# ishovkun/poroelasticity-dealii

Hardware: AMD Instinct MI355X
Metric: DoF-updates/sec in assemble+SpMV per fixed-stress iter (higher is better)
Workload: dtype f64

## Files before the change

poroelasticity_dealii_amd/csrc/common.hpp:

```cpp
#pragma once
#include <hip/hip_runtime.h>
#include <cstdint>
#include <cstdio>
#include <map>
#include <memory>
#include <type_traits>
#include <stdexcept>
#include <string>
#include <list>
#include <vector>
#include "../../include/poroel_hip.h"
#include "fdm_tables.hpp"
#include "cell_field.hpp"

namespace poro {

#define PORO_HIP(x)                                                                                   \
  do { hipError_t e_ = (x); if (e_ != hipSuccess) throw poro::Error(std::string(#x) + " -> " + hipGetErrorString(e_)); } while (0)

template <class T> struct DevBuf {
  T *p = nullptr; size_t n = 0;
  DevBuf() = default; DevBuf(const DevBuf &) = delete; DevBuf &operator=(const DevBuf &) = delete;
  ~DevBuf() { release(); }
  void release() { if (p) (void)hipFree(p); p = nullptr; n = 0; }
// ... 43 lines not shown
};
struct FdmDist : SlabLayout {
  bool built = false;
  FdmDir last;
  DevBuf<double> sendbuf, recvbuf, tz1, tz2; std::vector<double> hsend, hrecv;
  DevBuf<FdmWindow> windows;
};

struct FdmuDir { int n = 0; bool reg_form = false, split = false, blk = false; int n_even = 0; int blk_kk[2] = {0, 0}, blk_nch[2] = {0, 0}, blk_mb[2] = {0, 0} ; DevBuf<double> fwd, bwd, lam; };
struct FdmU : SlabLayout {
              int dim = 0; int nn[3] = {1, 1, 1}; double coef[3][3] = {}; FdmuDir dir[3][3]; FdmuDir last_global[3]; bool built = false, single = false;
              int fix[3][3][2] = {};
              bool dist = false; DevBuf<double> sendbuf, recvbuf, tz1, tz2;
              bool line = false; DevBuf<double> line_coef, line_fac; };
struct FdmoPlans;
struct FdmOct {
  bool built = false; int nt = 0;
  int n[3] = {1, 1, 1}, h[3] = {1, 1, 1}; int hxp = 2;
  int64_t co_stride = 0, n_oct = 0;
  double coef[3][3] = {};
  DevBuf<double> fwd[3][3][2], bwd[3][3][2], lam[3][3][2];
  DevBuf<float> fwd32[3][3][2], bwd32[3][3][2];
  DevBuf<double> g, z, t;
  DevBuf<double> gz_part; int gz_n = 0;
  std::vector<double> h_lam[3][3][2];
  DevBuf<double> bxy;
  int no = 8;
  int nc = 3;
  bool planar = false;
  int own_z = 0;
// ... 2 lines not shown
    bool on = false; int n_ranks = 1, rank = 0;
    int ng = 0, hzg = 0;
    bool zboth = false; DevBuf<int64_t> dst2;
    int np = 2, nb = 12;
    int cw = 64, nchunk = 0, cps = 0, chunk0 = 0, my_chunks = 0;
    int64_t scols = 0;
    int own = 0, nl = 0, max_own = 0, max_nl = 0, rows_back = 0;
    int64_t recv_off = 0;
    DevBuf<int64_t> row_in;
    DevBuf<int64_t> row_out; DevBuf<int32_t> row_kz;
    DevBuf<double> buf, tz;
  } slab;
  std::shared_ptr<FdmoPlans> plans;
  struct ScalarTable { double a, kappa; DevBuf<double> t; };
  std::list<ScalarTable> scalar_tables;
};
struct FdmQ1 { FdmScalar nodal; FdmOct fused; };
struct SsorLevels { DevBuf<int32_t> fwd_rows, bwd_rows; std::vector<int64_t> fwd_off, bwd_off; bool built = false; };
struct CsrDev {
  int64_t n = 0, nnz = 0;
  DevBuf<int64_t> rp; DevBuf<int32_t> col; DevBuf<int64_t> diag_pos;
  int lanes_per_row = 8;
  SsorLevels ssor;
};

struct ConsDev {
  int64_t n = 0, n_masters = 0;
  DevBuf<int32_t> dof, master; DevBuf<int64_t> ptr; DevBuf<double> weight, inhom;
  DevBuf<int32_t> t_master, t_dof; DevBuf<int64_t> t_ptr; DevBuf<double> t_weight;
  DevBuf<uint8_t> inert;
// ... 125 lines not shown

namespace poro {

inline bool box_fast_u(const poro_ctx *c) { return c->box.enabled && !c->mod.kind; }
inline bool moduli_structured_applies(const poro_ctx *c) {
  return c->box.enabled && c->dim == 3 && (c->k_u == 1 || c->k_u == 2) && c->mod.kind == 1 && c->operator_mode == PORO_OP_MATRIX_FREE && c->mf_variant == 1 && !c->comm.multi() &&
         c->comm.part.n_ranks <= 1;
}
inline bool moduli_structured(const poro_ctx *c) { return c->moduli_op == PORO_MODULI_OP_STRUCTURED && c->mod.planes.p && moduli_structured_applies(c); }

void la_fill(hipStream_t s, double *x, double v, int64_t n);
void la_nodal_interp(hipStream_t s, const int64_t *ptr, const int32_t *col, const double *w, int64_t n_rows, int ncomp, const double *in, double *out, int lanes = 1);
void la_two_level_combine(hipStream_t s, const int64_t *ptr, const int32_t *col, const double *w, int64_t n_rows, int ncomp, const double *zc, const double *g, const double *dinv, const uint8_t *inert, double omega, double *z, int lanes = 1);
void la_copy_many(hipStream_t s, int count, double *const *dst, const double *const *src, const int64_t *n);
void la_post(hipStream_t s, Mailbox *mb, unsigned long long seq, const double *src, int n, const PcgScalars *sc);
void la_copy(hipStream_t s, double *y, const double *x, int64_t n);
void la_axpy(hipStream_t s, double *y, double a, const double *x, int64_t n);
void la_add_range(hipStream_t s, double *y, const double *x, int64_t n);
void la_add_two_ranges(hipStream_t s, double *y0, const double *x0, double *y1, const double *x1, int64_t n);
void la_dot_partials(hipStream_t s, const double *a, const double *b, int64_t n, double *partials , const PcgScalars *gate = nullptr );
void la_norm_partials(hipStream_t s, const double *a, int64_t n, double *partials_l2, double *partials_inf);
void la_reduce_finish(hipStream_t s, const double *partials, int n_sets, double *red , int max_not_sum_mask);
void la_csr_spmv(hipStream_t s, const CsrDev &A, const double *val, const double *x, double *y);
void la_csr_residual(hipStream_t s, const CsrDev &A, const double *M, const double *K, double kappa, const double *t, const double *p,
                     const double *src, double *R);
void la_pressure_tmp(hipStream_t s, double *t, const double *ev, const double *ev0, const double *p, const double *p_old, double c1, double c2, int64_t n);
void la_jacobian(hipStream_t s, double *J, const double *M, const double *K, double a, double kappa, int64_t nnz);
void la_ifc_pack(hipStream_t s, const IfcDev &I, const double *v);
void la_ifc_sum(hipStream_t s, const IfcDev &I, double *v);
void la_csr_diag(hipStream_t s, const CsrDev &A, const double *val, double *diag);
// ... 97 lines not shown
void fdmu_line_factor(hipStream_t s, int ku, int ncomp, const FdmuLineArgs &a, double *fac );
void fdmu_line_solve(hipStream_t s, int ku, int ncomp, const FdmuLineArgs &a, const double *fac, double *v );
bool fdmo_usable(int dim, const int nn[3]);
void fdmo_init(FdmOct &O, const int nn[3], const double coef[3][3], hipStream_t s);
void fdmo_init_slab(FdmOct &O, const int nn[3], const double coef[3][3], int rank, const std::vector<int> &node_layers, bool has_upper, hipStream_t s);
void fdmo_init_per_direction(FdmOct &O, const int nn[3], const double coef[3][3], const FdmFormDecision &D, hipStream_t s);
void fdmo_upload_dir(FdmOct &O, int comp, int dir, const LineTables &T);
void fdmo_finalize(FdmOct &O);
void fdmo_apply(hipStream_t s, const FdmOct &O, const double *g_oct, double *z_oct, double *scratch_oct, const PcgScalars *gate = nullptr, hipEvent_t *ev  = nullptr,
                double *gz_part  = nullptr,
                int precision  = PORO_FDM_FP64,
                const PcgStopTest &stop = PcgStopTest{} );
bool fdmo_scalar_usable(int dim, const int nn[3]);
void fdmo_scalar_init(FdmOct &O, const int nn[3], hipStream_t s);
void fdmo_scalar_upload_dir(FdmOct &O, int dir, const LineTables &T);
void fdmo_scalar_apply(hipStream_t s, FdmOct &O, double a, double kappa, const double *g, double *z, const PcgScalars *gate = nullptr);
void fdmo_scalar_apply_many(hipStream_t s, FdmOct &O, double a, double kappa, int nb, const double *const *g, double *const *z, const PcgScalars *gate = nullptr);
void la_residual_norms_many(hipStream_t s, int nb, const double *const *y, const double *const *b, int64_t n, double *partials, const uint8_t *mask = nullptr);
void fdmo_scalar_init_slab(FdmOct &O, const int nn[3], int rank, const std::vector<int> &node_layers, hipStream_t s);
void fdmo_scalar_slab_pass(hipStream_t s, FdmOct &O, int pass, double a, double kappa, const double *in, double *out);
bool fdmo_planar_usable(int dim, const int nn[3]);
void fdmo_init_planar(FdmOct &O, const int nn[3], const double coef[3][3], hipStream_t s, bool split = true );
void fdmo_upload_dir_planar(FdmOct &O, int comp, int dir, const LineTables &T);
void fdmo_apply_planar(hipStream_t s, const FdmOct &O, const double *g_q, double *z_q, const PcgScalars *gate = nullptr, const PcgStopTest &stop = PcgStopTest{} );
void fdmo_from_nodal(hipStream_t s, const FdmOct &O, const double *v_nodal, double *q_oct);
void fdmo_to_nodal(hipStream_t s, const FdmOct &O, const double *r_oct, double *v_nodal);
void fdmo_init_residual(hipStream_t s, const FdmOct &O, double *g_oct, const double *Ax, const double *b, const uint8_t *inert);
void fdmo_first_direction(hipStream_t s, const FdmOct &O, double *d, const double *g_oct, const double *z_oct, double *partials );
void fdmo_update_g(hipStream_t s, const FdmOct &O, PcgScalars *sc, int parity, double *g_oct, const double *h, const uint8_t *inert, const double *partials_dh, double *partials_out , const double *red = nullptr);
void fdmo_update_d(hipStream_t s, const FdmOct &O, PcgScalars *sc, int parity, int it, double *x, double *d, const double *z_oct, const double *partials_in , const double *red = nullptr,
                   bool gz_from_pass = false ,
                   bool stream_x = false ,
// ... 19 lines not shown
```

poroelasticity_dealii_amd/csrc/ctx.hip:

```cpp
#include <dlfcn.h>
#include <rccl/rccl.h>
#include <algorithm>
#include <array>
#include <chrono>
#include <cmath>
#include <cstdlib>
#include <cstring>
#include <functional>
#include <thread>
#include <unordered_map>
#include "common.hpp"
#include "ctx_internal.hpp"

using namespace poro;
using namespace poro::ctx_detail;

namespace {
void lifting_from_wh(poro_ctx *c) {
  la_fill(c->stream, c->lift_u.p, 0.0, c->n_u);
  la_axpy(c->stream, c->lift_u.p, -1.0, c->wh_u.p, c->n_u);
}

void throw_unless_close(poro_ctx *c, double *a, const double *b, int64_t n, double rel_tol, const char *what) {
  hipStream_t s = c->stream;
// ... 313 lines not shown
  bool distribute_inhom = true;
};

const uint8_t *proj_inert(poro_ctx *c) { return c->cons_p.hanging.p ? c->cons_p.hanging.p : c->cons_p.inert.p; }

bool q1_stencil(poro_ctx *c) { return c->operator_mode == PORO_OP_MATRIX_FREE && c->box.enabled; }

bool solve_q1_direct(poro_ctx *c, double a, double kappa, int n, const double *const *b, double *const *x, double *y_scratch, bool batched,
                     const poro_solver_opts *opts, poro_solve_info *info, Q1Set set = Q1Set::free_ends, const uint8_t *mask = nullptr, const double *kap = nullptr, int kap_ncomp = 0) {
  hipStream_t s = c->stream;
  const double *y[3];
  for (int e = 0; e < n; ++e) y[e] = y_scratch + (size_t)e * c->n_p;
  const auto t0 = std::chrono::steady_clock::now();
  if (batched) {
    Timed tm(c, "precondition_p_fdm");
    fdmo_scalar_apply_many(s, c->q1_free.fused, a, kappa, n, b, x);
  } else {
    const double kk[3] = {kappa, kappa, kappa};
    for (int e = 0; e < n; ++e) { if (kap) fdm_precondition_p_layered(c, a, b[e], x[e], set); else fdm_precondition_p(c, a, kk, b[e], x[e], set); }
  }
  for (int e = 0; e < n; ++e) {
    {
      Timed tm(c, "apply_p_stencil");
      if (kap) p_stencil_apply_var(s, c->dim, c->box, a, kap, kap_ncomp, x[e], const_cast<double *>(y[e]));
      else p_stencil_apply(s, c->dim, c->box, a, kappa, x[e], const_cast<double *>(y[e]));
    }
    exchange_add(c, const_cast<double *>(y[e]), c->n_p, c->comm.part.plane_p);
  }
  la_residual_norms_many(s, n, y, b, owned(c, c->n_p, c->comm.part.plane_p), c->partials.p, mask);
  pcg_scalars_sum(s, c->partials.p, 2 * n, c->red.p);
  allreduce_sum(c, c->red.p, 2 * n);
  post_and_wait(c, c->red.p, 2 * n);
  bool all = true;
  for (int e = 0; e < n; ++e) {
    const double res = std::sqrt(c->mailbox->vals[2 * e]), bn = std::sqrt(c->mailbox->vals[2 * e + 1]);
    const bool ok = res <= std::max(opts->abs_tol, opts->rel_tol * bn);
    all = all && ok;
    if (!info) continue;
    info[e] = poro_solve_info{};
    info[e].iterations = 0;
    info[e].converged = ok ? 1 : 0;
    info[e].initial_residual = bn;
    info[e].final_residual = res;
    info[e].operator_applications = 1;
    info[e].seconds = std::chrono::duration<double>(std::chrono::steady_clock::now() - t0).count() / n;
  }
  return all;
// ... 332 lines not shown
    PORO_HIP(hipMemcpyAsync(host, vec(c, which), n * sizeof(double), hipMemcpyDeviceToHost, c->stream)); PORO_HIP(hipStreamSynchronize(c->stream)); return 0;
  });
}
int poro_vec_fill(poro_ctx *c, int which, double v) { return guarded([&] { PORO_HIP(hipSetDevice(c->device)); la_fill(c->stream, vec(c, which), v, vec_len(c, which)); return 0; }); }
int poro_vec_copy(poro_ctx *c, int dst, int src) {
  return guarded([&] { PORO_HIP(hipSetDevice(c->device)); if (vec_len(c, dst) != vec_len(c, src)) throw Error("vector length mismatch"); la_copy(c->stream, vec(c, dst), vec(c, src), vec_len(c, dst)); return 0; });
}
int poro_vec_axpy(poro_ctx *c, int y, double a, int x) {
  return guarded([&] { PORO_HIP(hipSetDevice(c->device)); if (vec_len(c, y) != vec_len(c, x)) throw Error("vector length mismatch"); la_axpy(c->stream, vec(c, y), a, vec(c, x), vec_len(c, y)); return 0; });
}
int poro_vec_norm(poro_ctx *c, int which, double *l2, double *linf) {
  return guarded([&] {
    PORO_HIP(hipSetDevice(c->device));
    const int64_t n = vec_len(c, which), plane = is_u_vec(which) ? c->comm.part.plane_u : c->comm.part.plane_p;
    la_norm_partials(c->stream, vec(c, which), owned(c, n, plane), c->partials.p, c->partials.p + kMaxPartials);
    la_reduce_finish(c->stream, c->partials.p, 2, c->red.p, 2);
    allreduce_sum(c, c->red.p, 1);
    post_and_wait(c, c->red.p, 2);
    if (l2) *l2 = std::sqrt(c->mailbox->vals[0]); if (linf) *linf = c->mailbox->vals[1]; return 0;
  });
}

int poro_state_save(poro_ctx *c) {
  return guarded([&] {
    PORO_HIP(hipSetDevice(c->device));
    std::vector<double *> dst; std::vector<const double *> src; std::vector<int64_t> len;
    for (auto &kv : c->vec) { DevBuf<double> &d = c->vec_saved[kv.first]; if (d.n != kv.second.n) d.alloc(kv.second.n); dst.push_back(d.p); src.push_back(kv.second.p); len.push_back((int64_t)kv.second.n); }
    la_copy_many(c->stream, (int)dst.size(), dst.data(), src.data(), len.data());
    PORO_HIP(hipStreamSynchronize(c->stream)); return 0;
  });
}
int poro_state_restore(poro_ctx *c) {
  return guarded([&] {
// ... 105 lines not shown
    PORO_HIP(hipSetDevice(c->device));
    hipStream_t s = c->stream; double *R = vec(c, PORO_VEC_RESIDUAL_P);
    const double *src = c->grav.flux_on() ? c->grav.src_p.p : c->src_local.p;
    {
      Timed tm(c, "pressure_residual");
      la_pressure_tmp(s, c->tmp_p.p, vec(c, PORO_VEC_EPSV), vec(c, PORO_VEC_EPSV0), vec(c, PORO_VEC_P), vec(c, PORO_VEC_P_OLD), c->mat.biot_alpha / dt, 1. / c->mat.biot_M / dt, c->n_p);
      if (c->operator_mode == PORO_OP_MATRIX_FREE && c->box.enabled) {
        if (c->perm.kind) p_residual_stencil_var(s, c->dim, c->box, c->perm.lattice.p, c->perm.ncomp, c->tmp_p.p, vec(c, PORO_VEC_P), src, R);
        else p_residual_stencil(s, c->dim, c->box, c->mat.k_over_mu, c->tmp_p.p, vec(c, PORO_VEC_P), src, R);
      } else la_csr_residual(s, c->Ap, c->Mp.p, c->Kp.p, c->perm.kind ? 1.0 : c->mat.k_over_mu, c->tmp_p.p, vec(c, PORO_VEC_P), src, R);
    }
    la_cons_reduce(s, c->cons_p, R);
    exchange_add(c, R, c->n_p, c->comm.part.plane_p);
    if (c->n_pdir) la_mask_zero(s, R, c->pdir_mask.p, c->n_p);
    la_dot_partials(s, R, R, owned(c, c->n_p, c->comm.part.plane_p), c->partials.p);
    la_reduce_finish(s, c->partials.p, 1, c->red.p, 0);
    allreduce_sum(c, c->red.p, 1);
    post_and_wait(c, c->red.p, 1);
    if (l2) *l2 = std::sqrt(c->mailbox->vals[0]);
    return 0;
  });
}

int poro_pres_apply_boundary_values(poro_ctx *c) {
  return guarded([&] {
    PORO_HIP(hipSetDevice(c->device));
    if (c->n_pdir) la_set_constrained(c->stream, vec(c, PORO_VEC_P), c->pdir_mask.p, c->pdir_val.p, c->n_p);
    if (c->n_pdir && c->cons_p.n) {
      la_cons_expand(c->stream, c->cons_p, vec(c, PORO_VEC_P), true);
      la_set_constrained(c->stream, vec(c, PORO_VEC_P), c->pdir_mask.p, c->pdir_val.p, c->n_p);
    }
    return 0;
  });
// ... 267 lines not shown
```

poroelasticity_dealii_amd/csrc/ctx_comm.hip:

```cpp
#include <dlfcn.h>
#include <rccl/rccl.h>
#include <algorithm>
#include <array>
#include <chrono>
#include <cmath>
#include <cstdlib>
#include <cstring>
#include <functional>
#include <thread>
#include <unordered_map>
#include "common.hpp"
#include "ctx_internal.hpp"

using namespace poro;
using namespace poro::ctx_detail;

namespace poro {
namespace ctx_detail {
thread_local std::string g_err;

Rccl g_rccl;
void Rccl::load() {
  if (lib) return;
  lib = dlopen("librccl.so.1", RTLD_NOW | RTLD_GLOBAL);
// ... 27 lines not shown
  }
}
static void isolate_sampled_dispatch(poro_ctx *c) {
  if (c->timing_stride <= 1) return;
  hipEvent_t m = event_get(c); (void)hipEventRecord(m, c->stream); c->event_pool.push_back(m);
}
Timer *begin_sampled_dispatch(poro_ctx *c, const char *family) {
  if (!c->timing) return nullptr;
  Timer *t = &c->timers[family];
  if (!t->sample(c->timing_stride)) return nullptr;
  isolate_sampled_dispatch(c);
  return t;
}


void post_and_wait(poro_ctx *c, const double *dev_src, int n, const PcgScalars *sc) {
  if (n > 16) throw Error("post_and_wait: at most 16 scalars");
  const unsigned long long want = ++c->mb_seq;
  la_post(c->stream, c->mailbox, want, dev_src, n, sc);
  PORO_HIP(hipGetLastError());
  const auto t0 = std::chrono::steady_clock::now(); unsigned spins = 0;
  while (__atomic_load_n(const_cast<unsigned long long *>(&c->mailbox->seq), __ATOMIC_ACQUIRE) != want) {
    __builtin_ia32_pause();
    if ((++spins & 0xfffff) == 0) {
      const hipError_t q = hipStreamQuery(c->stream);
      if (q != hipSuccess && q != hipErrorNotReady) throw Error(std::string("device failed while the host waited for its answer: ") + hipGetErrorString(q));
      if (q == hipSuccess && __atomic_load_n(const_cast<unsigned long long *>(&c->mailbox->seq), __ATOMIC_ACQUIRE) != want) throw Error("mailbox: the stream drained without publishing the expected sequence number");
      if (std::chrono::duration<double>(std::chrono::steady_clock::now() - t0).count() > 600.0) throw Error("mailbox: no answer from the device within 600 s");
    }
  }
}

void build_interface(poro_ctx *c, IfcDev &I, const int64_t *ptr, const int32_t *dof, int64_t n, int64_t n_owned) {
  const poro_partition &pt = c->comm.part; const int nn = pt.n_neighbours;
// ... 222 lines not shown
```

poroelasticity_dealii_amd/csrc/ctx_internal.hpp:

```cpp
#pragma once
#include <rccl/rccl.h>
#include <functional>
#include <string>
#include <vector>
#include "common.hpp"
#include "whole_faces.hpp"
#include "fdm_tables.hpp"

namespace poro {
namespace ctx_detail {

extern thread_local std::string g_err;
inline int ipow(int b, int e) { int r = 1; while (e--) r *= b; return r; }
template <class F> int guarded(F &&f) {
  try { return f(); }
  catch (const std::exception &e) { g_err = e.what(); return -1; }
}
template <class F> void for_each_colour(poro_ctx *c, F &&fn) {
  for (size_t k = 0; k + 1 < c->color_off.size(); ++k)
    fn(c->color_cells.p + c->color_off[k], c->color_off[k + 1] - c->color_off[k]);
}

struct Rccl {
  void *lib = nullptr;
// ... 23 lines not shown
  Timer *t = begin_sampled_dispatch(c, family);
  if (!t) return launch(nullptr, nullptr);
  hipEvent_t e0 = event_get(c), e1 = event_get(c);
  auto r = launch(e0, e1);
  t->pending.emplace_back(e0, e1);
  t->launches++;
  return r;
}
struct EventPair {
  poro_ctx *c; hipEvent_t e0, e1;
  explicit EventPair(poro_ctx *c_) : c(c_), e0(event_get(c_)), e1(event_get(c_)) {}
  ~EventPair() { c->event_pool.push_back(e0); c->event_pool.push_back(e1); }
  EventPair(const EventPair &) = delete; EventPair &operator=(const EventPair &) = delete;
};
void post_and_wait(poro_ctx *c, const double *dev_src, int n, const PcgScalars *sc = nullptr);

void setup_general_partition(poro_ctx *c, const poro_desc *d);
void exchange_planes(poro_ctx *c, const double *send_lo, const double *send_hi, int64_t plane);
void exchange_add(poro_ctx *c, double *v, int64_t n, int64_t plane);
void allreduce_sum(poro_ctx *c, double *dev, int n);
void allreduce_sum_vec(poro_ctx *c, double *dev, int64_t n, const char *timer);
int64_t owned(poro_ctx *c, int64_t n, int64_t plane);
AsmArgs asm_args(poro_ctx *c);
MfArgs mf_args(poro_ctx *c);
void mf_operator(poro_ctx *c, const double *x, double *y, bool constrained);
void mfg_operator(poro_ctx *c, const double *x, double *y, bool constrained);
void build_spatial_cells(poro_ctx *c);
void assemble_loads_u(poro_ctx *c);
void sync_moduli_planes(poro_ctx *c);
void hybrid_enable(poro_ctx *c);
// ... 76 lines not shown
```

poroelasticity_dealii_amd/csrc/ctx_prec.hip:

```cpp
#include <dlfcn.h>
#include <rccl/rccl.h>
#include <algorithm>
#include <array>
#include <chrono>
#include <cmath>
#include <cstdlib>
#include <cstring>
#include <functional>
#include <new>
#include <optional>
#include <thread>
#include <unordered_map>
#include "common.hpp"
#include "ctx_internal.hpp"
#include "perm_line.hpp"
#include "moduli_line.hpp"

using namespace poro;
using namespace poro::ctx_detail;

namespace poro {
namespace ctx_detail {
bool fdm_p_supported(poro_ctx *c) {
  if (!c->lines.on) return false;
// ... 58 lines not shown
  F.windows.upload(W);
  F.built = true;
}
void build_fdm_q1(poro_ctx *c, Q1Set which) {
  const bool fixed = which == Q1Set::fixed_ends;
  FdmQ1 &T = q1_set(c, which);
  if (T.nodal.built) return;
  if (fixed) {
    if (!fdm_pj_supported(c)) throw Error("PORO_PREC_FDM with prescribed pressures needs a uniform box or tensor-product grid on one rank whose prescribed set is a union of whole faces");
    if (c->timing) c->timers["fdm_pj_build"].enqueued += 1;
  } else if (!fdm_p_supported(c)) throw Error("PORO_PREC_FDM needs a uniform box (poro_desc.box.enabled) and, when partitioned, an initialised communicator");
  T.nodal.dim = c->dim;
  const bool multi = !fixed && c->comm.multi();
  int np3[3] = {c->lines.n[0] + 1, c->lines.n[1] + 1, c->dim == 3 ? c->lines.n[2] + 1 : 1};
  const bool fused = !multi && fdmo_scalar_usable(c->dim, np3) && !std::getenv("PORO_FDM_P_UNFUSED");
  if (fused) fdmo_scalar_init(T.fused, np3, c->stream);
  for (int d = 0; d < c->dim; ++d) {
    const std::vector<double> &hcell = c->lines.hcell[d]; const bool lo = fixed && c->pdir_face[d][0], hi = fixed && c->pdir_face[d][1];
    upload_dir(T.nodal.dir[d], c->lines.uniform && !lo && !hi ? q1_eig((int)hcell.size(), hcell[0]) : line_tables(1, hcell, lo, hi), fused ? &T.fused : nullptr, d);
  }
  if (!multi) T.fused.built = fused;
  if (c->fdm_t1.n < (size_t)c->n_p) { c->fdm_t1.alloc(c->n_p); c->fdm_t2.alloc(c->n_p); }
  if (multi) build_fdm_dist(c, np3);
  T.nodal.built = true;
}
void alltoall_blocks(poro_ctx *c, double *send, double *recv, int64_t blk, bool self_in_place) {
  Comm &cm = c->comm; const int N = cm.part.n_ranks, r = cm.part.rank;
  Timed tm(c, "alltoall");
  if (!self_in_place) PORO_HIP(hipMemcpyAsync(recv + (size_t)r * blk, send + (size_t)r * blk, blk * sizeof(double), hipMemcpyDeviceToDevice, c->stream));
  if (N <= 1) return;
  if (cm.nccl_comm) {
// ... 3 lines not shown
      PORO_NCCL(g_rccl.Send(send + (size_t)q * blk, blk, ncclFloat64, q, comm, c->stream));
      PORO_NCCL(g_rccl.Recv(recv + (size_t)q * blk, blk, ncclFloat64, q, comm, c->stream));
    }
    PORO_NCCL(g_rccl.GroupEnd());
  } else if (cm.sr) {
    FdmDist &F = c->fdm_dist; if ((int64_t)F.hsend.size() < blk) { F.hsend.resize(blk); F.hrecv.resize(blk); }
    for (int step = 0; step < N; ++step) {
      const int q = ((step - r) % N + N) % N;
      if (q == r) continue;
      PORO_HIP(hipMemcpyAsync(F.hsend.data(), send + (size_t)q * blk, blk * sizeof(double), hipMemcpyDeviceToHost, c->stream)); PORO_HIP(hipStreamSynchronize(c->stream));
      cm.sr(F.hsend.data(), F.hrecv.data(), blk, q, cm.user);
      PORO_HIP(hipMemcpyAsync(recv + (size_t)q * blk, F.hrecv.data(), blk * sizeof(double), hipMemcpyHostToDevice, c->stream)); PORO_HIP(hipStreamSynchronize(c->stream));
    }
  } else throw Error("partitioned context without a communicator");
}
void fdm_precondition_p(poro_ctx *c, double a, const double k[3], const double *g, double *z, Q1Set which) {
  Timed tm(c, "precondition_p_fdm");
  hipStream_t s = c->stream;
  const bool fixed = which == Q1Set::fixed_ends, isotropic = k[0] == k[1] && k[1] == k[2];
  FdmQ1 &T = q1_set(c, which);
  if (fixed || !c->comm.multi()) {
    std::optional<Timed> tf; if (fixed) tf.emplace(c, "precondition_p_fdm_fixed_ends");
    if (T.fused.built && isotropic) fdmo_scalar_apply(s, T.fused, a, k[0], g, z);
    else fdm_apply(s, T.nodal, a, k, g, z, c->fdm_t1.p, c->fdm_t2.p);
    return;
  }
  if (T.fused.built && T.fused.slab.on && isotropic) {
    FdmOct &O = T.fused; auto &S = O.slab; double *send = S.buf.p, *recv = S.buf.p + S.recv_off;
    fdmo_scalar_slab_pass(s, O, 1, a, k[0], g, S.buf.p);
    alltoall_blocks(c, send, recv, (int64_t)S.max_own * S.scols, true);
    fdmo_scalar_slab_pass(s, O, 2, a, k[0], S.buf.p, S.tz.p);
    fdmo_slab_scatter_pack(s, O, nullptr);
    alltoall_blocks(c, send, recv, (int64_t)S.max_nl * S.scols, true);
    fdmo_scalar_slab_pass(s, O, 3, a, k[0], S.buf.p, z);
    return;
  }
  FdmDist &F = c->fdm_dist; const FdmScalar &L = T.nodal;
  const int dim = c->dim, N = F.n_ranks, r = F.rank, last = dim - 1;
// ... 374 lines not shown
```

poroelasticity_dealii_amd/csrc/kernels_fdmo.hip:

```cpp
#include "common.hpp"
#include "fdm_tables.hpp"
#include "device_reduce.hpp"
#include <hip/hip_ext.h>
#include <cmath>
#include <cstdlib>
#include <limits>
#include <mutex>
#include <set>
#include <type_traits>

namespace poro {
namespace {

typedef double v4d __attribute__((ext_vector_type(4)));
typedef float v4f __attribute__((ext_vector_type(4)));

struct OctDims { int nx, ny, nz, hx, hy, hz, hxp; int64_t co; int no, own_z, nc; int split; int part[8]; };

__device__ __forceinline__ void bfly_fwd(double (&v)[8], const bool (&centre)[3]) {
#pragma unroll
  for (int bit = 0; bit < 3; ++bit) {
    const int m = 1 << bit;
#pragma unroll
    for (int i = 0; i < 8; ++i) if (!(i & m)) {
// ... 422 lines not shown
    int tr, tc; tile_of(a, tr, tc, kColsSecond);
    if (a == NL + 1 && !heavy) continue;
#pragma unroll
    for (int q = 0; q < 4; ++q) {
      const int r = 16 * tr + 4 * q + kq, cc = 16 * tc + j;
      if (MODE == 0 && f_slab_io == 1) { if (r < R && cc < C && b < P.store_planes) out[slab_at(r * (int)P.row_stride + cc)] = acc[a][q]; }
      else if (r < R && cc < C) out[base_out + (int64_t)r * P.row_stride + cc] = acc[a][q];
    }
  }
  if (P.stamps) {
    __builtin_amdgcn_s_waitcnt(0); __syncthreads(); stamp(5);
    if (tid == 0) { unsigned hw, xcc; asm volatile("s_getreg_b32 %0, hwreg(HW_REG_HW_ID)" : "=s"(hw)); asm volatile("s_getreg_b32 %0, hwreg(HW_REG_XCC_ID)" : "=s"(xcc)); P.stamps[(int64_t)blockIdx.x * 8 + 6] = hw; P.stamps[(int64_t)blockIdx.x * 8 + 7] = xcc; }
  }
}


template <int NT, int MODE, bool GZ = false>
__global__ void __launch_bounds__(64 * pass_waves<NT>())
k_fdmo_pass_f32(OctPass P, const double *in, double *out) {
  static_assert(!GZ || MODE == 1, "g . z comes out of pass 2");
  typedef PassGeom<NT> Gm;
  constexpr int NW = pass_waves<NT>();
  constexpr bool EXTRA = NT > NW;
  constexpr int XT = NT - 1;
  constexpr int NL = (MODE == 1 && EXTRA) ? NW : NT;
  constexpr bool CORNER = EXTRA && MODE != 1;
  constexpr int NACC = NL + (EXTRA ? 1 : 0) + (CORNER ? 1 : 0);
  constexpr bool kColsFirst = MODE == 0, kColsSecond = MODE == 2;
  constexpr int LD1 = kColsFirst ? Gm::LDA : Gm::LDB, LD2 = kColsSecond ? Gm::LDA : Gm::LDB;
  constexpr int NS = EXTRA ? 2 : 1;
// ... 683 lines not shown

bool fdmo_scalar_usable(int dim, const int nn[3]) { if (dim != 3) return false; for (int d = 0; d < 3; ++d) if (nn[d] > 16 * kFdmoMaxTiles || nn[d] < 2) return false; return true; }
void fdmo_scalar_init(FdmOct &O, const int nn[3], hipStream_t s) {
  form_geometry(O, nn, nullptr, 0, 1, s);
  O.t.alloc(3 * O.n_oct); O.t.zero(s);
}
void fdmo_scalar_upload_dir(FdmOct &O, int dir, const LineTables &T) {
  const int n = T.n; const std::vector<double> &S = T.S, &lam = T.lam;
  if (n != (O.slab.on && dir == 2 ? O.slab.ng : O.n[dir])) throw Error("fdmo_scalar_upload_dir: line length mismatch");
  std::vector<double> lp(16 * O.nt + 16, std::numeric_limits<double>::infinity());
  for (int m = 0; m < n; ++m) lp[m] = lam[m];
  O.h_lam[0][dir][0] = lp; O.lam[0][dir][0].upload(lp);
  O.fwd[0][dir][0].upload(pack_fragments<double>(O.nt, 4 * O.nt, n, n, [&](int r, int cc) { return S[(size_t)cc * n + r]; })); O.bwd[0][dir][0].upload(pack_fragments<double>(O.nt, 4 * O.nt, n, n, [&](int r, int cc) { return S[(size_t)r * n + cc]; }));
}
static const double *scalar_table(hipStream_t s, FdmOct &O, double a, double kappa);
void fdmo_scalar_apply(hipStream_t s, FdmOct &O, double a, double kappa, const double *g, double *z, const PcgScalars *gate) {
  const double *gs[1] = {g}; double *zs[1] = {z};
  fdmo_scalar_apply_many(s, O, a, kappa, 1, gs, zs, gate);
}
void fdmo_scalar_apply_many(hipStream_t s, FdmOct &O, double a, double kappa, int nb, const double *const *g, double *const *z, const PcgScalars *gate) {
  if (nb < 1 || nb > 3) throw Error("fdmo_scalar_apply_many: 1..3 right-hand sides");
  const Form F = scalar_form(O, nb, kappa, scalar_table(s, O, a, kappa));
  const double *const in[3] = {g[0], O.t.p, O.t.p}; double *const out[3] = {O.t.p, O.t.p, z[0]};
  for (int k = 0; k < 3; ++k) {
    OctPass P = plan_pass(F, k + 1);
    P.gate = gate;
    for (int c = 0; c < nb; ++c) { P.in_blk[c] = g[c]; P.out_blk[c] = z[c]; }
    P.use_in_off = k == 0; P.use_out_off = k == 2;
    launch_pass_nt(s, O.nt, PassVariant::General, P, nb * P.nblk, in[k], out[k]);
  }
}

static const double *scalar_table(hipStream_t s, FdmOct &O, double a, double kappa) {
  for (auto &T : O.scalar_tables) if (T.a == a && T.kappa == kappa) return T.t.p;
  const int hx = O.h[0], hy = O.h[1];
  if (O.scalar_tables.size() >= 8) { PORO_HIP(hipStreamSynchronize(s)); O.scalar_tables.pop_front(); }
  std::vector<double> Bt((size_t)hx * hy);
  const double inf = std::numeric_limits<double>::infinity();
  for (int my = 0; my < hy; ++my) for (int mx = 0; mx < hx; ++mx) {
    const double lx = O.h_lam[0][0][0][mx], ly = O.h_lam[0][1][0][my];
    Bt[(size_t)my * hx + mx] = (lx < 1e300 && ly < 1e300) ? a + kappa * (lx + ly) : inf;
  }
  O.scalar_tables.emplace_back(); auto &T = O.scalar_tables.back(); T.a = a; T.kappa = kappa; T.t.upload(Bt); return T.t.p;
}
void fdmo_scalar_slab_pass(hipStream_t s, FdmOct &O, int pass, double a, double kappa, const double *in, double *out) {
// ... 89 lines not shown
```

poroelasticity_dealii_amd/csrc/kernels_la.hip:

```cpp
#include "common.hpp"
#include "device_reduce.hpp"

namespace poro {
namespace {

__global__ void k_post(Mailbox *mb, unsigned long long seq, const double *src, int n, const PcgScalars *sc) {
  if ((int)threadIdx.x < n) mb->vals[threadIdx.x] = src[threadIdx.x];
  if (sc && threadIdx.x == 32) mb->sc = *sc;
  __threadfence_system();
  __syncthreads();
  if (threadIdx.x == 0) __hip_atomic_store(const_cast<unsigned long long *>(&mb->seq), seq, __ATOMIC_RELEASE, __HIP_MEMORY_SCOPE_SYSTEM);
}
__global__ void k_fill(double *x, double v, int64_t n) {
  for (int64_t i = (int64_t)blockIdx.x * kBlock + threadIdx.x; i < n; i += (int64_t)gridDim.x * kBlock) x[i] = v;
}
__global__ void k_axpy(double *y, double a, const double *x, int64_t n) {
  for (int64_t i = (int64_t)blockIdx.x * kBlock + threadIdx.x; i < n; i += (int64_t)gridDim.x * kBlock) y[i] += a * x[i];
}
__global__ void k_dot(const double *a, const double *b, int64_t n, double *partials, const PcgScalars *gate) {
  __shared__ double sh[4];
  if (pcg_gate_closed(gate)) return;
  double s = 0;
  for (int64_t i = (int64_t)blockIdx.x * kBlock + threadIdx.x; i < n; i += (int64_t)gridDim.x * kBlock) s += a[i] * b[i];
  s = block_sum(s, sh);
// ... 3 lines not shown
  __shared__ double sh[4];
  double s = 0, m = 0;
  for (int64_t i = (int64_t)blockIdx.x * kBlock + threadIdx.x; i < n; i += (int64_t)gridDim.x * kBlock) { const double v = a[i]; s += v * v; m = fmax(m, fabs(v)); }
  s = block_sum(s, sh); m = block_max(m, sh);
  store_partial(p2, s); store_partial(pinf, m);
}
__global__ void k_reduce_finish(const double *partials, int n_sets, double *red, int max_mask) {
  __shared__ double sh[4];
  for (int k = 0; k < n_sets; ++k) {
    const bool is_max = (max_mask >> k) & 1;
    double v = 0;
    for (int i = threadIdx.x; i < kMaxPartials; i += kBlock) { const double t = partials[k * kMaxPartials + i]; v = is_max ? fmax(v, t) : v + t; }
    v = is_max ? block_max(v, sh) : block_sum(v, sh);
    if (threadIdx.x == 0) red[k] = v;
  }
}

template <int L> __global__ void k_spmv(int64_t n, const int64_t *__restrict__ rp, const int32_t *__restrict__ col, const double *__restrict__ val,
                                        const double *__restrict__ x, double *__restrict__ y) {
  const int lane = threadIdx.x % L;
  const int64_t row = ((int64_t)blockIdx.x * kBlock + threadIdx.x) / L;
  if (row >= n) return;
  const int64_t b = rp[row], e = rp[row + 1];
  double s = 0;
  constexpr int U = 4;
  for (int64_t j0 = b + lane; j0 < e; j0 += (int64_t)L * U) {
    double v[U]; int32_t c[U];
#pragma unroll
    for (int u = 0; u < U; ++u) { const int64_t j = j0 + (int64_t)u * L; const bool ok = j < e; v[u] = ok ? val[j] : 0.0; c[u] = col[ok ? j : b]; }
#pragma unroll
// ... 354 lines not shown
    double rr = 0, bb = 0;
    for (int64_t i = (int64_t)blockIdx.x * kBlock + threadIdx.x; i < n; i += (int64_t)gridDim.x * kBlock) {
      if (MASKED && mask[i]) continue;
      const double bv = V.b[e][i], r = V.y[e][i] - bv; rr = fma(r, r, rr); bb = fma(bv, bv, bb);
    }
    rr = block_sum(rr, sh); bb = block_sum(bb, sh);
    store_partial(partials + (size_t)(2 * e) * kMaxPartials, rr); store_partial(partials + (size_t)(2 * e + 1) * kMaxPartials, bb);
  }
}
void la_residual_norms_many(hipStream_t s, int nb, const double *const *y, const double *const *b, int64_t n, double *partials, const uint8_t *mask) {
  ManyPairs V{}; for (int e = 0; e < nb; ++e) { V.y[e] = y[e]; V.b[e] = b[e]; }
  if (mask) hipLaunchKernelGGL(k_residual_norms_many<true>, reduce_grid(n), kBlock, 0, s, V, nb, n, partials, mask);
  else hipLaunchKernelGGL(k_residual_norms_many<false>, reduce_grid(n), kBlock, 0, s, V, nb, n, partials, mask);
}
void la_post(hipStream_t s, Mailbox *mb, unsigned long long seq, const double *src, int n, const PcgScalars *sc) { hipLaunchKernelGGL(k_post, 1, 64, 0, s, mb, seq, src, n, sc); }
void la_fill(hipStream_t s, double *x, double v, int64_t n) { if (n) hipLaunchKernelGGL(k_fill, grid_for(n), kBlock, 0, s, x, v, n); }
__global__ void k_copy(double *__restrict__ y, const double *__restrict__ x, int64_t n) {
  const int64_t n2 = n >> 1;
  double2 *y2 = reinterpret_cast<double2 *>(y); const double2 *x2 = reinterpret_cast<const double2 *>(x);
  for (int64_t i = (int64_t)blockIdx.x * kBlock + threadIdx.x; i < n2; i += (int64_t)gridDim.x * kBlock) y2[i] = x2[i];
  if ((n & 1) && blockIdx.x == 0 && threadIdx.x == 0) y[n - 1] = x[n - 1];
}
void la_copy(hipStream_t s, double *y, const double *x, int64_t n) {
  if (!n || y == x) return;
  if (((uintptr_t)y | (uintptr_t)x) & 15) { PORO_HIP(hipMemcpyAsync(y, x, n * sizeof(double), hipMemcpyDeviceToDevice, s)); return; }
  hipLaunchKernelGGL(k_copy, grid_for(n, 8), kBlock, 0, s, y, x, n);
}
struct CopyMany { double *dst[24]; const double *src[24]; int64_t n[24]; };
__global__ void __launch_bounds__(kBlock) k_copy_many(CopyMany V) {
  const int v = blockIdx.y; const int64_t n = V.n[v], n2 = n >> 1;
// ... 257 lines not shown
```

Before: 24.12 billion.

## Add strip-split FDM scalar passes for small grids and fuse reduce with mailbox post

Adds a strip variant of the fused FDM scalar preconditioner passes. When the number of work items falls below a fraction of the CU count, each block is split across several workgroups so that small problems can fill the GPU. Separately, on a single rank it merges the reduce-finish and mailbox-post kernels into one launch to cut per-reduction launch latency. The strip kernel adds code paths restricted to single-rank general passes, and there is a new launch counter in the timers.

```diff
diff --git a/poroelasticity_dealii_amd/csrc/common.hpp b/poroelasticity_dealii_amd/csrc/common.hpp
--- a/poroelasticity_dealii_amd/csrc/common.hpp
+++ b/poroelasticity_dealii_amd/csrc/common.hpp
@@ -81,6 +81,7 @@
               bool dist = false; DevBuf<double> sendbuf, recvbuf, tz1, tz2;
               bool line = false; DevBuf<double> line_coef, line_fac; };
 struct FdmoPlans;
+constexpr double kFdmoStripFill = 0.4;
 struct FdmOct {
   bool built = false; int nt = 0;
   int n[3] = {1, 1, 1}, h[3] = {1, 1, 1}; int hxp = 2;
@@ -113,6 +114,7 @@
   std::shared_ptr<FdmoPlans> plans;
   struct ScalarTable { double a, kappa; DevBuf<double> t; };
   std::list<ScalarTable> scalar_tables;
+  double strip_limit = 0;
 };
 struct FdmQ1 { FdmScalar nodal; FdmOct fused; };
 struct SsorLevels { DevBuf<int32_t> fwd_rows, bwd_rows; std::vector<int64_t> fwd_off, bwd_off; bool built = false; };
@@ -268,6 +270,7 @@
 void la_two_level_combine(hipStream_t s, const int64_t *ptr, const int32_t *col, const double *w, int64_t n_rows, int ncomp, const double *zc, const double *g, const double *dinv, const uint8_t *inert, double omega, double *z, int lanes = 1);
 void la_copy_many(hipStream_t s, int count, double *const *dst, const double *const *src, const int64_t *n);
 void la_post(hipStream_t s, Mailbox *mb, unsigned long long seq, const double *src, int n, const PcgScalars *sc);
+void la_reduce_post(hipStream_t s, const double *partials, int n_sets, double *red, int max_not_sum_mask, Mailbox *mb, unsigned long long seq);
 void la_copy(hipStream_t s, double *y, const double *x, int64_t n);
 void la_axpy(hipStream_t s, double *y, double a, const double *x, int64_t n);
 void la_add_range(hipStream_t s, double *y, const double *x, int64_t n);
@@ -395,8 +398,8 @@
 bool fdmo_scalar_usable(int dim, const int nn[3]);
 void fdmo_scalar_init(FdmOct &O, const int nn[3], hipStream_t s);
 void fdmo_scalar_upload_dir(FdmOct &O, int dir, const LineTables &T);
-void fdmo_scalar_apply(hipStream_t s, FdmOct &O, double a, double kappa, const double *g, double *z, const PcgScalars *gate = nullptr);
-void fdmo_scalar_apply_many(hipStream_t s, FdmOct &O, double a, double kappa, int nb, const double *const *g, double *const *z, const PcgScalars *gate = nullptr);
+int fdmo_scalar_apply(hipStream_t s, FdmOct &O, double a, double kappa, const double *g, double *z, const PcgScalars *gate = nullptr);
+int fdmo_scalar_apply_many(hipStream_t s, FdmOct &O, double a, double kappa, int nb, const double *const *g, double *const *z, const PcgScalars *gate = nullptr);
 void la_residual_norms_many(hipStream_t s, int nb, const double *const *y, const double *const *b, int64_t n, double *partials, const uint8_t *mask = nullptr);
 void fdmo_scalar_init_slab(FdmOct &O, const int nn[3], int rank, const std::vector<int> &node_layers, hipStream_t s);
 void fdmo_scalar_slab_pass(hipStream_t s, FdmOct &O, int pass, double a, double kappa, const double *in, double *out);
diff --git a/poroelasticity_dealii_amd/csrc/ctx.hip b/poroelasticity_dealii_amd/csrc/ctx.hip
--- a/poroelasticity_dealii_amd/csrc/ctx.hip
+++ b/poroelasticity_dealii_amd/csrc/ctx.hip
@@ -351,7 +351,7 @@
   const auto t0 = std::chrono::steady_clock::now();
   if (batched) {
     Timed tm(c, "precondition_p_fdm");
-    fdmo_scalar_apply_many(s, c->q1_free.fused, a, kappa, n, b, x);
+    count_strip_launches(c, fdmo_scalar_apply_many(s, c->q1_free.fused, a, kappa, n, b, x));
   } else {
     const double kk[3] = {kappa, kappa, kappa};
     for (int e = 0; e < n; ++e) { if (kap) fdm_precondition_p_layered(c, a, b[e], x[e], set); else fdm_precondition_p(c, a, kk, b[e], x[e], set); }
@@ -365,9 +365,7 @@
     exchange_add(c, const_cast<double *>(y[e]), c->n_p, c->comm.part.plane_p);
   }
   la_residual_norms_many(s, n, y, b, owned(c, c->n_p, c->comm.part.plane_p), c->partials.p, mask);
-  pcg_scalars_sum(s, c->partials.p, 2 * n, c->red.p);
-  allreduce_sum(c, c->red.p, 2 * n);
-  post_and_wait(c, c->red.p, 2 * n);
+  post_sums_and_wait(c, c->partials.p, 2 * n, 0, 2 * n);
   bool all = true;
   for (int e = 0; e < n; ++e) {
     const double res = std::sqrt(c->mailbox->vals[2 * e]), bn = std::sqrt(c->mailbox->vals[2 * e + 1]);
@@ -730,9 +728,7 @@
     PORO_HIP(hipSetDevice(c->device));
     const int64_t n = vec_len(c, which), plane = is_u_vec(which) ? c->comm.part.plane_u : c->comm.part.plane_p;
     la_norm_partials(c->stream, vec(c, which), owned(c, n, plane), c->partials.p, c->partials.p + kMaxPartials);
-    la_reduce_finish(c->stream, c->partials.p, 2, c->red.p, 2);
-    allreduce_sum(c, c->red.p, 1);
-    post_and_wait(c, c->red.p, 2);
+    post_sums_and_wait(c, c->partials.p, 2, 2, 1);
     if (l2) *l2 = std::sqrt(c->mailbox->vals[0]); if (linf) *linf = c->mailbox->vals[1]; return 0;
   });
 }
@@ -868,9 +864,7 @@
     exchange_add(c, R, c->n_p, c->comm.part.plane_p);
     if (c->n_pdir) la_mask_zero(s, R, c->pdir_mask.p, c->n_p);
     la_dot_partials(s, R, R, owned(c, c->n_p, c->comm.part.plane_p), c->partials.p);
-    la_reduce_finish(s, c->partials.p, 1, c->red.p, 0);
-    allreduce_sum(c, c->red.p, 1);
-    post_and_wait(c, c->red.p, 1);
+    post_sums_and_wait(c, c->partials.p, 1, 0, 1);
     if (l2) *l2 = std::sqrt(c->mailbox->vals[0]);
     return 0;
   });
diff --git a/poroelasticity_dealii_amd/csrc/ctx_comm.hip b/poroelasticity_dealii_amd/csrc/ctx_comm.hip
--- a/poroelasticity_dealii_amd/csrc/ctx_comm.hip
+++ b/poroelasticity_dealii_amd/csrc/ctx_comm.hip
@@ -65,10 +65,26 @@
 }
 
 
+static void mailbox_wait(poro_ctx *c, unsigned long long want);
 void post_and_wait(poro_ctx *c, const double *dev_src, int n, const PcgScalars *sc) {
   if (n > 16) throw Error("post_and_wait: at most 16 scalars");
   const unsigned long long want = ++c->mb_seq;
   la_post(c->stream, c->mailbox, want, dev_src, n, sc);
+  mailbox_wait(c, want);
+}
+void post_sums_and_wait(poro_ctx *c, const double *partials, int n_sets, int max_mask, int n_allreduce) {
+  if (n_sets > 16) throw Error("post_sums_and_wait: at most 16 scalars");
+  if (c->comm.multi()) {
+    la_reduce_finish(c->stream, partials, n_sets, c->red.p, max_mask);
+    allreduce_sum(c, c->red.p, n_allreduce);
+    post_and_wait(c, c->red.p, n_sets);
+    return;
+  }
+  const unsigned long long want = ++c->mb_seq;
+  la_reduce_post(c->stream, partials, n_sets, c->red.p, max_mask, c->mailbox, want);
+  mailbox_wait(c, want);
+}
+static void mailbox_wait(poro_ctx *c, unsigned long long want) {
   PORO_HIP(hipGetLastError());
   const auto t0 = std::chrono::steady_clock::now(); unsigned spins = 0;
   while (__atomic_load_n(const_cast<unsigned long long *>(&c->mailbox->seq), __ATOMIC_ACQUIRE) != want) {
diff --git a/poroelasticity_dealii_amd/csrc/ctx_internal.hpp b/poroelasticity_dealii_amd/csrc/ctx_internal.hpp
--- a/poroelasticity_dealii_amd/csrc/ctx_internal.hpp
+++ b/poroelasticity_dealii_amd/csrc/ctx_internal.hpp
@@ -61,6 +61,8 @@
   EventPair(const EventPair &) = delete; EventPair &operator=(const EventPair &) = delete;
 };
 void post_and_wait(poro_ctx *c, const double *dev_src, int n, const PcgScalars *sc = nullptr);
+void post_sums_and_wait(poro_ctx *c, const double *partials, int n_sets, int max_mask, int n_allreduce);
+void count_strip_launches(poro_ctx *c, int n);
 
 void setup_general_partition(poro_ctx *c, const poro_desc *d);
 void exchange_planes(poro_ctx *c, const double *send_lo, const double *send_hi, int64_t plane);
diff --git a/poroelasticity_dealii_amd/csrc/ctx_prec.hip b/poroelasticity_dealii_amd/csrc/ctx_prec.hip
--- a/poroelasticity_dealii_amd/csrc/ctx_prec.hip
+++ b/poroelasticity_dealii_amd/csrc/ctx_prec.hip
@@ -96,7 +96,11 @@
   const bool multi = !fixed && c->comm.multi();
   int np3[3] = {c->lines.n[0] + 1, c->lines.n[1] + 1, c->dim == 3 ? c->lines.n[2] + 1 : 1};
   const bool fused = !multi && fdmo_scalar_usable(c->dim, np3) && !std::getenv("PORO_FDM_P_UNFUSED");
-  if (fused) fdmo_scalar_init(T.fused, np3, c->stream);
+  if (fused) {
+    fdmo_scalar_init(T.fused, np3, c->stream);
+    const char *strips = std::getenv("PORO_FDMO_SCALAR_STRIPS");
+    T.fused.strip_limit = (strips ? std::max(0.0, std::atof(strips)) : kFdmoStripFill) * c->n_cus;
+  }
   for (int d = 0; d < c->dim; ++d) {
     const std::vector<double> &hcell = c->lines.hcell[d]; const bool lo = fixed && c->pdir_face[d][0], hi = fixed && c->pdir_face[d][1];
     upload_dir(T.nodal.dir[d], c->lines.uniform && !lo && !hi ? q1_eig((int)hcell.size(), hcell[0]) : line_tables(1, hcell, lo, hi), fused ? &T.fused : nullptr, d);
@@ -130,6 +134,7 @@
     }
   } else throw Error("partitioned context without a communicator");
 }
+void count_strip_launches(poro_ctx *c, int n) { if (n) c->timers["fdm_q1_strip_launches"].enqueued += n; }
 void fdm_precondition_p(poro_ctx *c, double a, const double k[3], const double *g, double *z, Q1Set which) {
   Timed tm(c, "precondition_p_fdm");
   hipStream_t s = c->stream;
@@ -137,7 +142,7 @@
   FdmQ1 &T = q1_set(c, which);
   if (fixed || !c->comm.multi()) {
     std::optional<Timed> tf; if (fixed) tf.emplace(c, "precondition_p_fdm_fixed_ends");
-    if (T.fused.built && isotropic) fdmo_scalar_apply(s, T.fused, a, k[0], g, z);
+    if (T.fused.built && isotropic) count_strip_launches(c, fdmo_scalar_apply(s, T.fused, a, k[0], g, z));
     else fdm_apply(s, T.nodal, a, k, g, z, c->fdm_t1.p, c->fdm_t2.p);
     return;
   }
diff --git a/poroelasticity_dealii_amd/csrc/kernels_fdmo.hip b/poroelasticity_dealii_amd/csrc/kernels_fdmo.hip
--- a/poroelasticity_dealii_amd/csrc/kernels_fdmo.hip
+++ b/poroelasticity_dealii_amd/csrc/kernels_fdmo.hip
@@ -460,6 +460,93 @@
   }
 }
 
+template <int NT, int MODE>
+__global__ void __launch_bounds__(64 * NT)
+k_fdmo_strip(OctPass P, const double *in, double *out) {
+  typedef PassGeom<NT> Gm;
+  constexpr bool kColsFirst = MODE == 0, kColsSecond = MODE == 2;
+  constexpr int LD1 = MODE == 1 ? 16 : (kColsFirst ? Gm::LDA : Gm::LDB), LD2 = MODE == 1 ? 16 : (kColsSecond ? Gm::LDA : Gm::LDB);
+  constexpr int PADC = MODE == 1 ? 16 : Gm::PADN, KKP = Gm::KKP;
+  extern __shared__ double L[];
+  if (pcg_gate_closed(P.gate)) return;
+  const int tid = threadIdx.x, lane = tid & 63, w = __builtin_amdgcn_readfirstlane(tid >> 6);
+  const int j = lane & 15, kq = lane >> 4;
+  const int item = MODE == 1 ? (int)blockIdx.x : (int)blockIdx.x / NT, s = MODE == 1 ? 0 : (int)blockIdx.x - item * NT;
+  const int co = item / P.nblk, b = item - co * P.nblk;
+  const int R = P.R, C = MODE == 1 ? min(P.C, P.pl - b * P.C) : P.C;
+  if ((MODE == 0 && 16 * s >= C) || (MODE == 2 && 16 * s >= R)) return;
+  const int64_t base = (int64_t)co * P.co_stride + (int64_t)b * P.blk_stride;
+  const int64_t base_in = P.use_in_off ? (int64_t)b * P.blk_stride : base, base_out = P.use_out_off ? (int64_t)b * P.blk_stride : base;
+  if (P.use_in_off) in = P.in_blk[co];
+  if (P.use_out_off) out = P.out_blk[co];
+  const int f1 = MODE == 1 ? w : s;
+  const double *__restrict__ T1 = static_cast<const double *>(P.T1[co][0]) + (int64_t)f1 * KKP * 64 + lane, *__restrict__ T2 = static_cast<const double *>(P.T2[co][0]) + (int64_t)w * KKP * 64 + lane;
+  double t1[KKP], t2[KKP];
+#pragma unroll
+  for (int kk = 0; kk < KKP; ++kk) t1[kk] = T1[kk * 64];
+  {
+    constexpr int TOT = Gm::PADN * PADC, PER = TOT / (64 * NT);
+    static_assert(TOT % (64 * NT) == 0, "staging loop");
+    double stage[PER];
+#pragma unroll
+    for (int u = 0; u < PER; ++u) { const int e = tid + u * 64 * NT, r = e / PADC, cc = e - r * PADC; stage[u] = (r < R && cc < C) ? in[base_in + (int64_t)r * P.row_stride + cc] : 0.0; }
+#pragma unroll
+    for (int u = 0; u < PER; ++u) { const int e = tid + u * 64 * NT, r = e / PADC, cc = e - r * PADC; L[r * LD1 + cc] = stage[u]; }
+  }
+#pragma unroll
+  for (int kk = 0; kk < KKP; ++kk) t2[kk] = T2[kk * 64];
+  __syncthreads();
+  v4d acc = v4d{0, 0, 0, 0};
+  {
+    const double *La = kColsFirst ? L + (16 * w + j) * LD1 + kq : L + kq * LD1 + (MODE == 1 ? 0 : 16 * w) + j;
+#pragma unroll
+    for (int kk = 0; kk < KKP; ++kk) {
+      if (kk < KKP - 3 || kk < P.kk1) {
+        const double d = kColsFirst ? La[4 * kk] : La[4 * kk * LD1];
+        acc = kColsFirst ? __builtin_amdgcn_mfma_f64_16x16x4f64(d, t1[kk], acc, 0, 0, 0) : __builtin_amdgcn_mfma_f64_16x16x4f64(t1[kk], d, acc, 0, 0, 0);
+      }
+    }
+  }
+  __syncthreads();
+  {
+    const int tr = MODE == 2 ? s : w, tc = MODE == 0 ? s : (MODE == 2 ? w : 0);
+    if constexpr (MODE == 1) {
+      const double *lamz = P.lam_z[co][0]; const double czc = P.cz[co];
+      const double bxy = P.bxy[min(b * P.C + j, P.pl - 1)];
+#pragma unroll
+      for (int q = 0; q < 4; ++q) {
+        const double den = fma(czc, lamz[16 * w + 4 * q + kq], bxy);
+        double r = __builtin_amdgcn_rcp(den);
+        r = den < 1e300 ? fma(r, fma(-den, r, 1.0), r) : 0.0;
+        L[(16 * tr + 4 * q + kq) * LD2 + 16 * tc + j] = acc[q] * r;
+      }
+    } else {
+#pragma unroll
+      for (int q = 0; q < 4; ++q) L[(16 * tr + 4 * q + kq) * LD2 + 16 * tc + j] = acc[q];
+    }
+  }
+  acc = v4d{0, 0, 0, 0};
+  __syncthreads();
+  {
+    const double *La = kColsSecond ? L + (16 * s + j) * LD2 + kq : L + kq * LD2 + 16 * s + j;
+#pragma unroll
+    for (int kk = 0; kk < KKP; ++kk) {
+      if (kk < KKP - 3 || kk < P.kk2) {
+        const double d = kColsSecond ? La[4 * kk] : La[4 * kk * LD2];
+        acc = kColsSecond ? __builtin_amdgcn_mfma_f64_16x16x4f64(d, t2[kk], acc, 0, 0, 0) : __builtin_amdgcn_mfma_f64_16x16x4f64(t2[kk], d, acc, 0, 0, 0);
+      }
+    }
+  }
+  {
+    const int tr = MODE == 2 ? s : w, tc = MODE == 0 ? s : (MODE == 2 ? w : 0);
+#pragma unroll
+    for (int q = 0; q < 4; ++q) {
+      const int r = 16 * tr + 4 * q + kq, cc = 16 * tc + j;
+      if (r < R && cc < C) out[base_out + (int64_t)r * P.row_stride + cc] = acc[q];
+    }
+  }
+}
+
 
 template <int NT, int MODE, bool GZ = false>
 __global__ void __launch_bounds__(64 * pass_waves<NT>())
@@ -1173,21 +1260,54 @@
   O.fwd[0][dir][0].upload(pack_fragments<double>(O.nt, 4 * O.nt, n, n, [&](int r, int cc) { return S[(size_t)cc * n + r]; })); O.bwd[0][dir][0].upload(pack_fragments<double>(O.nt, 4 * O.nt, n, n, [&](int r, int cc) { return S[(size_t)r * n + cc]; }));
 }
 static const double *scalar_table(hipStream_t s, FdmOct &O, double a, double kappa);
-void fdmo_scalar_apply(hipStream_t s, FdmOct &O, double a, double kappa, const double *g, double *z, const PcgScalars *gate) {
+int fdmo_scalar_apply(hipStream_t s, FdmOct &O, double a, double kappa, const double *g, double *z, const PcgScalars *gate) {
   const double *gs[1] = {g}; double *zs[1] = {z};
-  fdmo_scalar_apply_many(s, O, a, kappa, 1, gs, zs, gate);
-}
-void fdmo_scalar_apply_many(hipStream_t s, FdmOct &O, double a, double kappa, int nb, const double *const *g, double *const *z, const PcgScalars *gate) {
+  return fdmo_scalar_apply_many(s, O, a, kappa, 1, gs, zs, gate);
+}
+template <int NT, int MODE> void launch_strip_one(hipStream_t s, int n_wg, const OctPass &P, const double *in, double *out) {
+  constexpr unsigned lds = (unsigned)(PassGeom<NT>::PADN * (MODE == 1 ? 16 : PassGeom<NT>::LDMAX) * sizeof(double));
+  if (lds > 64 * 1024) {
+    static std::mutex mu; static std::set<int> done; int dev = 0; PORO_HIP(hipGetDevice(&dev));
+    std::lock_guard<std::mutex> lk(mu);
+    if (!done.count(dev)) { PORO_HIP(hipFuncSetAttribute(reinterpret_cast<const void *>(k_fdmo_strip<NT, MODE>), hipFuncAttributeMaxDynamicSharedMemorySize, (int)lds)); done.insert(dev); }
+  }
+  hipLaunchKernelGGL((k_fdmo_strip<NT, MODE>), dim3((unsigned)n_wg), dim3(64 * NT), lds, s, P, in, out);
+}
+template <int NT> void launch_strip(hipStream_t s, const OctPass &P, int n_items, const double *in, double *out) {
+  if (P.mode == 0) launch_strip_one<NT, 0>(s, n_items * NT, P, in, out);
+  else if (P.mode == 2) launch_strip_one<NT, 2>(s, n_items * NT, P, in, out);
+  else launch_strip_one<NT, 1>(s, n_items, P, in, out);
+}
+void launch_strip_nt(hipStream_t s, int nt, const OctPass &P, int n_items, const double *in, double *out) {
+  if (variant_of_flags(P) != PassVariant::General || P.slab_z || P.slab_io || P.row_in || P.no_shift || P.bxy_cmul || P.stop.gg_part || P.gz_part || P.stamps) throw Error("fdmo: the strip form serves the scalar passes of one rank only");
+  switch (nt) {
+    case 2: launch_strip<2>(s, P, n_items, in, out); break;
+    case 3: launch_strip<3>(s, P, n_items, in, out); break;
+    case 4: launch_strip<4>(s, P, n_items, in, out); break;
+    case 5: launch_strip<5>(s, P, n_items, in, out); break;
+    case 6: launch_strip<6>(s, P, n_items, in, out); break;
+    case 7: launch_strip<7>(s, P, n_items, in, out); break;
+    case 8: launch_strip<8>(s, P, n_items, in, out); break;
+    default: throw Error("fdmo: lines of more than 128 entries");
+  }
+}
+int fdmo_scalar_apply_many(hipStream_t s, FdmOct &O, double a, double kappa, int nb, const double *const *g, double *const *z, const PcgScalars *gate) {
   if (nb < 1 || nb > 3) throw Error("fdmo_scalar_apply_many: 1..3 right-hand sides");
   const Form F = scalar_form(O, nb, kappa, scalar_table(s, O, a, kappa));
   const double *const in[3] = {g[0], O.t.p, O.t.p}; double *const out[3] = {O.t.p, O.t.p, z[0]};
+  int strips = 0;
   for (int k = 0; k < 3; ++k) {
     OctPass P = plan_pass(F, k + 1);
     P.gate = gate;
     for (int c = 0; c < nb; ++c) { P.in_blk[c] = g[c]; P.out_blk[c] = z[c]; }
     P.use_in_off = k == 0; P.use_out_off = k == 2;
-    launch_pass_nt(s, O.nt, PassVariant::General, P, nb * P.nblk, in[k], out[k]);
-  }
+    const bool strip = O.nt >= 2 && !O.slab.on && (double)nb * P.nblk < O.strip_limit && g[0] != O.t.p && z[0] != O.t.p;
+    if (!strip) { launch_pass_nt(s, O.nt, PassVariant::General, P, nb * P.nblk, in[k], out[k]); continue; }
+    if (k == 1) { P.C = 16; P.blk_stride = 16; P.nblk = (P.pl + 15) / 16; }
+    launch_strip_nt(s, O.nt, P, nb * P.nblk, in[k], out[k]);
+    ++strips;
+  }
+  return strips;
 }
 
 static const double *scalar_table(hipStream_t s, FdmOct &O, double a, double kappa) {
diff --git a/poroelasticity_dealii_amd/csrc/kernels_la.hip b/poroelasticity_dealii_amd/csrc/kernels_la.hip
--- a/poroelasticity_dealii_amd/csrc/kernels_la.hip
+++ b/poroelasticity_dealii_amd/csrc/kernels_la.hip
@@ -41,6 +41,19 @@
     v = is_max ? block_max(v, sh) : block_sum(v, sh);
     if (threadIdx.x == 0) red[k] = v;
   }
+}
+__global__ void k_reduce_post(const double *partials, int n_sets, double *red, int max_mask, Mailbox *mb, unsigned long long seq) {
+  __shared__ double sh[4];
+  for (int k = 0; k < n_sets; ++k) {
+    const bool is_max = (max_mask >> k) & 1;
+    double v = 0;
+    for (int i = threadIdx.x; i < kMaxPartials; i += kBlock) { const double t = partials[k * kMaxPartials + i]; v = is_max ? fmax(v, t) : v + t; }
+    v = is_max ? block_max(v, sh) : block_sum(v, sh);
+    if (threadIdx.x == 0) { red[k] = v; mb->vals[k] = v; }
+  }
+  __threadfence_system();
+  __syncthreads();
+  if (threadIdx.x == 0) __hip_atomic_store(const_cast<unsigned long long *>(&mb->seq), seq, __ATOMIC_RELEASE, __HIP_MEMORY_SCOPE_SYSTEM);
 }
 
 template <int L> __global__ void k_spmv(int64_t n, const int64_t *__restrict__ rp, const int32_t *__restrict__ col, const double *__restrict__ val,
@@ -425,6 +438,9 @@
   else hipLaunchKernelGGL(k_residual_norms_many<false>, reduce_grid(n), kBlock, 0, s, V, nb, n, partials, mask);
 }
 void la_post(hipStream_t s, Mailbox *mb, unsigned long long seq, const double *src, int n, const PcgScalars *sc) { hipLaunchKernelGGL(k_post, 1, 64, 0, s, mb, seq, src, n, sc); }
+void la_reduce_post(hipStream_t s, const double *partials, int n_sets, double *red, int max_mask, Mailbox *mb, unsigned long long seq) {
+  hipLaunchKernelGGL(k_reduce_post, 1, kBlock, 0, s, partials, n_sets, red, max_mask, mb, seq);
+}
 void la_fill(hipStream_t s, double *x, double v, int64_t n) { if (n) hipLaunchKernelGGL(k_fill, grid_for(n), kBlock, 0, s, x, v, n); }
 __global__ void k_copy(double *__restrict__ y, const double *__restrict__ x, int64_t n) {
   const int64_t n2 = n >> 1;
```

Result: faster. 24.40 billion (median of 6 runs) (+1.2%).
